# haesungpyun/seoul_tourism_recommendation_NGCF

Measured on AMD Instinct MI355X. Metric: NGCF 3-layer forward: propagated edges/sec + achieved HBM GB/s, d=128, higher is better.
Workload: dtype f32

## Files before the change

### seoul_tourism_recommendation_ngcf_amd/csrc/dense.hip

```cpp
#include "common.h"
#include <type_traits>

#ifndef NGCF_DC
#define NGCF_DC 16
#endif
#define NGCF_KC (2 * NGCF_DC)

typedef float f32x16 __attribute__((ext_vector_type(16)));
typedef float f32x4 __attribute__((ext_vector_type(4)));

__device__ __forceinline__ void pack_bias2(const float *__restrict__ b1, const float *__restrict__ b2, int d_out, int DOP,
                                           float *__restrict__ bias2)
{
    for (int j = threadIdx.x; j < DOP; j += 256) bias2[j] = j < d_out ? (b1[j] + b1[j]) + b2[j] : 0.f;
}

template <class T> __device__ __forceinline__ T tile_row(T base, int r, int lh) { return base + (r & 3) + 8 * (r >> 2) + 4 * lh; }

struct DenseAct {
    float leaky, drop_p, keep_scale;
    uint32_t drop_thr;
    uint64_t drop_seed;
    const float *drop_mask;
    int64_t ldm, n_rows;
// ... 156 lines not shown
        const int kl = idx / 32, w = idx % 32;
        Wt[((int64_t)chunk * NGCF_KC + kl) * DOP + g * 32 + w] = tile[kl][w];
    }
    if (blockIdx.x == 0) pack_bias2(b1, b2, d_out, DOP, bias2);
}

#ifndef NGCF_DENSE_WAVES_PER_EU
#define NGCF_DENSE_WAVES_PER_EU 1
#endif
template <int RW, int CW, int NT, bool ALIGNED, bool FAST>
__global__ __launch_bounds__(256, NGCF_DENSE_WAVES_PER_EU) void layer_dense_kernel(const float *__restrict__ LE, int64_t ldLE,
                                                          const float *__restrict__ Es, int64_t ldE, int64_t n_rows,
                                                          int d_in, int d_out, const float *__restrict__ Wt,
                                                          const float *__restrict__ bias2, int n_chunks,
                                                          float leaky, float drop_p, uint64_t drop_seed_in,
                                                          const float *__restrict__ drop_mask, int64_t ldm,
                                                          float *__restrict__ carry, int64_t ldc,
                                                          float *__restrict__ norm, int64_t ldn)
{
    const uint64_t drop_seed = drop_p > 0.f ? resolve_seed(drop_seed_in) : drop_seed_in;
    constexpr int BM = 32 * RW;
    constexpr int WCOLS = 32 * NT * CW;
    constexpr int XLD = NGCF_KC + 4;
    constexpr bool DB = WCOLS <= 128;
    constexpr int NBUF = DB ? 2 : 1;
    constexpr int SQ = NGCF_DC / 4;
    constexpr int RPP = 256 / SQ;
    constexpr int RR = (BM + RPP - 1) / RPP;
    constexpr int WF4 = NGCF_KC * WCOLS / 4;
    constexpr int WN = (WF4 + 255) / 256;
    __shared__ float Xs[NBUF * BM * XLD];
    __shared__ float Ws[NBUF * NGCF_KC * WCOLS];
    __shared__ float ssq[BM * CW];

    const int tid = threadIdx.x;
    const int wave = tid >> 6, lane = tid & 63;
    const int rw = wave / CW, cw = wave % CW;
    const int li = lane & 31, lh = lane >> 5;
    const int64_t row0 = (int64_t)blockIdx.x * BM;

    f32x16 acc[NT];
#pragma unroll
    for (int t = 0; t < NT; ++t)
#pragma unroll
        for (int r = 0; r < 16; ++r) acc[t][r] = 0.f;

    const int sq = tid % SQ;
    const int sr = tid / SQ;
    f32x4 xle[RR], xe[RR], wreg[WN];

    auto load_chunk = [&](int chunk) {
        const int c0 = chunk * NGCF_DC + sq * 4;
        if constexpr (FAST) {
            const int d4 = (d_in + 3) & ~3;
            const int cc = c0 < d4 ? c0 : d4 - 4;
            const bool k0 = c0 < d_in, k1 = c0 + 1 < d_in, k2 = c0 + 2 < d_in, k3 = c0 + 3 < d_in;
#pragma unroll
            for (int rr = 0; rr < RR; ++rr) {
                int64_t grow = row0 + (sr + rr * RPP) % BM;
                grow = grow < n_rows ? grow : n_rows - 1;
                f32x4 a = *reinterpret_cast<const f32x4 *>(LE + grow * ldLE + cc);
                f32x4 b = *reinterpret_cast<const f32x4 *>(Es + grow * ldE + cc);
                a.x = k0 ? a.x : 0.f; a.y = k1 ? a.y : 0.f; a.z = k2 ? a.z : 0.f; a.w = k3 ? a.w : 0.f;
                b.x = k0 ? b.x : 0.f; b.y = k1 ? b.y : 0.f; b.z = k2 ? b.z : 0.f; b.w = k3 ? b.w : 0.f;
                xle[rr] = a;
                xe[rr] = b;
            }
            const f32x4 *srcw = reinterpret_cast<const f32x4 *>(Wt + (int64_t)chunk * NGCF_KC * WCOLS);
#pragma unroll
            for (int i = 0; i < WN; ++i)
                if (WF4 % 256 == 0 || tid + i * 256 < WF4) wreg[i] = srcw[tid + i * 256];
            return;
        }
#pragma unroll
        for (int rr = 0; rr < RR; ++rr) {
            const int r = sr + rr * RPP;
            float le[4] = {0.f, 0.f, 0.f, 0.f}, e[4] = {0.f, 0.f, 0.f, 0.f};
            const int64_t grow = row0 + r;
            if (r < BM && grow < n_rows) {
                if (ALIGNED && c0 + 4 <= d_in) {
                    const float4 a = *reinterpret_cast<const float4 *>(LE + grow * ldLE + c0);
                    const float4 b = *reinterpret_cast<const float4 *>(Es + grow * ldE + c0);
                    le[0] = a.x; le[1] = a.y; le[2] = a.z; le[3] = a.w;
                    e[0] = b.x; e[1] = b.y; e[2] = b.z; e[3] = b.w;
                } else {
#pragma unroll
                    for (int q = 0; q < 4; ++q)
                        if (c0 + q < d_in) {
                            le[q] = LE[grow * ldLE + c0 + q];
                            e[q] = Es[grow * ldE + c0 + q];
                        }
                }
            }
            xle[rr] = f32x4{le[0], le[1], le[2], le[3]};
            xe[rr] = f32x4{e[0], e[1], e[2], e[3]};
        }
        const f32x4 *src = reinterpret_cast<const f32x4 *>(Wt + (int64_t)chunk * NGCF_KC * WCOLS);
#pragma unroll
        for (int i = 0; i < WN; ++i)
            if (WF4 % 256 == 0 || tid + i * 256 < WF4) wreg[i] = src[tid + i * 256];
    };
    auto store_chunk = [&](int buf) {
        float *X = Xs + buf * (BM * XLD);
#pragma unroll
        for (int rr = 0; rr < RR; ++rr) {
            const int r = sr + rr * RPP;
            if (r < BM) {
                const f32x4 a = xle[rr], b = xe[rr];
                *reinterpret_cast<f32x4 *>(X + r * XLD + sq * 4) = a + b;
                *reinterpret_cast<f32x4 *>(X + r * XLD + NGCF_DC + sq * 4) = a * b;
            }
        }
        f32x4 *dst = reinterpret_cast<f32x4 *>(Ws + buf * (NGCF_KC * WCOLS));
#pragma unroll
        for (int i = 0; i < WN; ++i)
            if (WF4 % 256 == 0 || tid + i * 256 < WF4) dst[tid + i * 256] = wreg[i];
    };
    auto compute_chunk = [&](int buf) {
        const float *X = Xs + buf * (BM * XLD) + (rw * 32 + li) * XLD + lh * 4;
        const float *W = Ws + buf * (NGCF_KC * WCOLS) + cw * (32 * NT) + li * NT;
#pragma unroll
        for (int kb = 0; kb < NGCF_KC / 8; ++kb) {
            const f32x4 a4 = *reinterpret_cast<const f32x4 *>(X + kb * 8);
#define NGCF_KSTEP(sx, aval)                                                                                   \
    {                                                                                                          \
        const float *wk = W + (kb * 8 + lh * 4 + sx) * WCOLS;                                                  \
        float bv[NT];                                                                                          \
        _Pragma("unroll") for (int t = 0; t < NT; ++t) bv[t] = wk[t];                                          \
        _Pragma("unroll") for (int t = 0; t < NT; ++t)                                                         \
            acc[t] = __builtin_amdgcn_mfma_f32_32x32x2f32(aval, bv[t], acc[t], 0, 0, 0);                       \
    }
            NGCF_KSTEP(0, a4.x) NGCF_KSTEP(1, a4.y) NGCF_KSTEP(2, a4.z) NGCF_KSTEP(3, a4.w)
#undef NGCF_KSTEP
        }
    };

    if (DB) {
        load_chunk(0);
        store_chunk(0);
        __syncthreads();
        for (int chunk = 0; chunk < n_chunks; ++chunk) {
            const bool more = chunk + 1 < n_chunks;
            if (more) load_chunk(chunk + 1);
            compute_chunk(chunk & 1);
            if (more) store_chunk((chunk + 1) & 1);
            __syncthreads();
        }
    } else {
        load_chunk(0);
        store_chunk(0);
        __syncthreads();
        for (int chunk = 0; chunk < n_chunks; ++chunk) {
            const bool more = chunk + 1 < n_chunks;
            if (more) load_chunk(chunk + 1);
            compute_chunk(0);
            __syncthreads();
            if (more) {
                store_chunk(0);
                __syncthreads();
            }
        }
    }

    const float keep_scale = drop_p > 0.f ? 1.f / (1.f - drop_p) : 1.f;
    const uint32_t drop_thr = msg_drop_thr(drop_p);
    float rowss[16];
#pragma unroll
    for (int r = 0; r < 16; ++r) rowss[r] = 0.f;
    if (!drop_mask && !(drop_p > 0.f)) {
#pragma unroll
        for (int t = 0; t < NT; ++t) {
            const int col = (cw * NT + t) * 32 + li;
            const float bz = bias2[col];
#pragma unroll
            for (int r = 0; r < 16; ++r) {
                float v = acc[t][r] + bz;
                v = v >= 0.f ? v : leaky * v;
                acc[t][r] = v;
                rowss[r] = fmaf(v, v, rowss[r]);
            }
        }
    } else {
#pragma unroll
        for (int t = 0; t < NT; ++t) {
            const int col = (cw * NT + t) * 32 + li;
            const float bz = bias2[col];
#pragma unroll
            for (int r = 0; r < 16; ++r) {
                float v = acc[t][r] + bz;
                v = v >= 0.f ? v : leaky * v;
                if (drop_mask) {
                    const int64_t grow = tile_row(row0 + rw * 32, r, lh);
                    v *= (grow < n_rows && col < d_out) ? drop_mask[grow * ldm + col] : 0.f;
                } else if (drop_p > 0.f) {
                    const int64_t grow = tile_row(row0 + rw * 32, r, lh);
                    v = msg_drop(v, drop_seed, grow, col, drop_thr, keep_scale);
                }
                acc[t][r] = v;
                rowss[r] = fmaf(v, v, rowss[r]);
            }
        }
    }
#pragma unroll
    for (int r = 0; r < 16; ++r) {
        float s = rowss[r];
        s += __shfl_xor(s, 1);
        s += __shfl_xor(s, 2);
        s += __shfl_xor(s, 4);
        s += __shfl_xor(s, 8);
        s += __shfl_xor(s, 16);
        rowss[r] = s;
    }
    if (CW > 1) {
        if (li == 0) {
#pragma unroll
            for (int r = 0; r < 16; ++r) {
                const int lr = tile_row(rw * 32, r, lh);
                ssq[lr * CW + cw] = rowss[r];
            }
        }
        __syncthreads();
#pragma unroll
        for (int r = 0; r < 16; ++r) {
            const int lr = tile_row(rw * 32, r, lh);
            float s = 0.f;
#pragma unroll
            for (int q = 0; q < CW; ++q) s += ssq[lr * CW + q];
            rowss[r] = s;
        }
    }
    if (row0 + BM <= n_rows && d_out == WCOLS) {
#pragma unroll
        for (int r = 0; r < 16; ++r) {
            const int64_t grow = tile_row(row0 + rw * 32, r, lh);
            const float inv = 1.f / fmaxf(sqrtf(rowss[r]), 1e-12f);
            float *nrow = norm + grow * ldn + cw * NT * 32 + li;
#pragma unroll
            for (int t = 0; t < NT; ++t) nrow[t * 32] = acc[t][r] * inv;
        }
        if (carry) {
#pragma unroll
            for (int r = 0; r < 16; ++r) {
                const int64_t grow = tile_row(row0 + rw * 32, r, lh);
                float *crow = carry + grow * ldc + cw * NT * 32 + li;
#pragma unroll
                for (int t = 0; t < NT; ++t) crow[t * 32] = acc[t][r];
            }
        }
        return;
    }
#pragma unroll
    for (int r = 0; r < 16; ++r) {
        const int64_t grow = tile_row(row0 + rw * 32, r, lh);
        if (grow >= n_rows) continue;
        const float nrm = fmaxf(sqrtf(rowss[r]), 1e-12f);
        const float inv = 1.f / nrm;
#pragma unroll
        for (int t = 0; t < NT; ++t) {
            const int col = (cw * NT + t) * 32 + li;
            if (col < d_out) {
                const float v = acc[t][r];
                if (carry) carry[grow * ldc + col] = v;
                norm[grow * ldn + col] = v * inv;
            }
        }
    }
}

constexpr int kResWaves = 8, kResWGs = 256;

typedef __bf16 bf16x8 __attribute__((ext_vector_type(8)));
typedef float f32x8 __attribute__((ext_vector_type(8)));

__device__ __forceinline__ void split3(f32x8 x, bf16x8 &h, bf16x8 &m, bf16x8 &l)
{
    h = __builtin_convertvector(x, bf16x8);
    const f32x8 r = x - __builtin_convertvector(h, f32x8);
    m = __builtin_convertvector(r, bf16x8);
    l = __builtin_convertvector(r - __builtin_convertvector(m, f32x8), bf16x8);
}

__global__ __launch_bounds__(256) void pack_weights_split_kernel(const float *__restrict__ W1, const float *__restrict__ b1,
                                                                 const float *__restrict__ W2, const float *__restrict__ b2,
                                                                 int d_in, int d_out, int n_chunks, bf16x8 *__restrict__ Whm,
                                                                 bf16x8 *__restrict__ Wl, float *__restrict__ bias2)
{
    const int idx = blockIdx.x * 256 + threadIdx.x;
    if (idx < n_chunks * 512) {
        const int lane = idx & 63, frag = idx >> 6, t = frag & 3, s = (frag >> 2) & 1, c = frag >> 3;
        const int col = t * 32 + (lane & 31), in0 = c * NGCF_DC + 8 * (lane >> 5);
        const float *w = (s ? W2 : W1) + (int64_t)col * d_in;
        f32x8 x;
#pragma unroll
        for (int j = 0; j < 8; ++j) x[j] = (col < d_out && in0 + j < d_in) ? w[in0 + j] : 0.f;
        bf16x8 h, m, l;
        split3(x, h, m, l);
        Whm[(frag * 2 + 0) * 64 + lane] = h;
        Whm[(frag * 2 + 1) * 64 + lane] = m;
        Wl[idx] = l;
    }
    if (blockIdx.x == 0) pack_bias2(b1, b2, d_out, 128, bias2);
}

template <bool SPLIT>
__device__ __forceinline__ void dense_persistent_tiles(const float *LE, int64_t ldLE, const float *Es, int64_t ldE, int64_t n_rows,
                                                       int d_in, int d_out, const f32x4 *w_lds, const bf16x8 *Wl, const float *bias2,
                                                       int n_chunks, float leaky, float drop_p, uint64_t drop_seed_in,
                                                       const float *drop_mask, int64_t ldm, float *carry, int64_t ldc, float *norm,
                                                       int64_t ldn)
{
    const uint64_t drop_seed = drop_p > 0.f ? resolve_seed(drop_seed_in) : drop_seed_in;
    constexpr int NT = 4, WCOLS = 128;
    constexpr int CA = SPLIT ? 8 : 4, CB = SPLIT ? 4 : 8;
    using AFrag = std::conditional_t<SPLIT, bf16x8[2][3], f32x4[4]>;
    constexpr int NL = SPLIT ? 8 : 1;
    extern __shared__ f32x4 Wres[];
    const int tid = threadIdx.x, wave = tid >> 6, lane = tid & 63;
    const int li = lane & 31, lh = lane >> 5;
    for (int i = tid; i < n_chunks * 1024; i += kResWaves * 64) Wres[i] = w_lds[i];
    __syncthreads();
    const int64_t n_tiles = (n_rows + 31) / 32;
    const int d4 = (d_in + 3) & ~3;
    float bz[NT];
#pragma unroll
    for (int t = 0; t < NT; ++t) bz[t] = bias2[t * 32 + li];
    const int last = n_chunks - 1;
    const int64_t tile_step = (int64_t)gridDim.x * kResWaves;
    auto row_of = [&](int64_t t) {
        int64_t g = t * 32 + li;
        return g < n_rows ? g : n_rows - 1;
    };
    auto fetch = [&](const float *le_row, const float *e_row, int c, f32x4 &la, f32x4 &lb, f32x4 &ea, f32x4 &eb) {
        const int ca = c * NGCF_DC + lh * CA;
        fetch_pieces(le_row, e_row, ca, ca + CB, d4, la, lb, ea, eb);
    };
    auto fetch_l = [&](int c, bf16x8 (&bl)[NL]) {
        if constexpr (SPLIT) {
#pragma unroll
            for (int f = 0; f < 8; ++f) bl[f] = Wl[(c * 8 + f) * 64 + lane];
        }
    };
    f32x4 la0, lb0, ea0, eb0, la1, lb1, ea1, eb1;
    bf16x8 bl0[NL], bl1[NL];
    auto fetch_tile = [&](int64_t t) {
        const int64_t g = row_of(t);
        fetch(LE + g * ldLE, Es + g * ldE, 0, la0, lb0, ea0, eb0);
        fetch(LE + g * ldLE, Es + g * ldE, last < 1 ? last : 1, la1, lb1, ea1, eb1);
    };
    fetch_l(0, bl0);
    int64_t tile = (int64_t)blockIdx.x * kResWaves + wave;
    fetch_tile(tile < n_tiles ? tile : 0);
    for (; tile < n_tiles; tile += tile_step) {
        const int64_t row0 = tile * 32;
        const int64_t grow_l = row_of(tile);
        const float *le_row = LE + grow_l * ldLE, *e_row = Es + grow_l * ldE;
        f32x16 acc[NT];
#pragma unroll
        for (int t = 0; t < NT; ++t)
#pragma unroll
            for (int r = 0; r < 16; ++r) acc[t][r] = 0.f;
        auto form = [&](int c, f32x4 la, f32x4 lb, f32x4 ea, f32x4 eb, AFrag &a) {
            const int ca = c * NGCF_DC + lh * CA;
            zero_tail(ca, ca + CB, d_in, la, lb, ea, eb);
            const f32x4 sa = la + ea, sb = lb + eb, pa = la * ea, pb = lb * eb;
            if constexpr (SPLIT) {
                split3(__builtin_shufflevector(sa, sb, 0, 1, 2, 3, 4, 5, 6, 7), a[0][0], a[0][1], a[0][2]);
                split3(__builtin_shufflevector(pa, pb, 0, 1, 2, 3, 4, 5, 6, 7), a[1][0], a[1][1], a[1][2]);
            } else {
                a[0] = sa, a[1] = sb, a[2] = pa, a[3] = pb;
            }
        };
        auto chunk_mfma = [&](int c, const AFrag &a, const bf16x8 (&bl)[NL]) {
            if constexpr (SPLIT) {
                const bf16x8 *wc = reinterpret_cast<const bf16x8 *>(Wres) + c * 1024 + lane;
#pragma unroll
                for (int s = 0; s < 2; ++s) {
                    const bf16x8 &ah = a[s][0], &am = a[s][1], &al = a[s][2];
#pragma unroll
                    for (int t = 0; t < NT; ++t) {
                        const bf16x8 bh = wc[((s * 4 + t) * 2 + 0) * 64], bm = wc[((s * 4 + t) * 2 + 1) * 64];
                        acc[t] = __builtin_amdgcn_mfma_f32_32x32x16_bf16(am, bm, acc[t], 0, 0, 0);
                        acc[t] = __builtin_amdgcn_mfma_f32_32x32x16_bf16(al, bh, acc[t], 0, 0, 0);
                        acc[t] = __builtin_amdgcn_mfma_f32_32x32x16_bf16(ah, bl[s * 4 + t], acc[t], 0, 0, 0);
                        acc[t] = __builtin_amdgcn_mfma_f32_32x32x16_bf16(am, bh, acc[t], 0, 0, 0);
                        acc[t] = __builtin_amdgcn_mfma_f32_32x32x16_bf16(ah, bm, acc[t], 0, 0, 0);
                        acc[t] = __builtin_amdgcn_mfma_f32_32x32x16_bf16(ah, bh, acc[t], 0, 0, 0);
                    }
                }
            } else {
                const float *wc = reinterpret_cast<const float *>(Wres) + li * NT + (int64_t)c * NGCF_KC * WCOLS;
#pragma unroll
                for (int kb = 0; kb < 4; ++kb) {
#pragma unroll
                    for (int sx = 0; sx < 4; ++sx) {
                        const f32x4 bv = *reinterpret_cast<const f32x4 *>(wc + (kb * 8 + lh * 4 + sx) * WCOLS);
                        acc[0] = __builtin_amdgcn_mfma_f32_32x32x2f32(a[kb][sx], bv.x, acc[0], 0, 0, 0);
                        acc[1] = __builtin_amdgcn_mfma_f32_32x32x2f32(a[kb][sx], bv.y, acc[1], 0, 0, 0);
                        acc[2] = __builtin_amdgcn_mfma_f32_32x32x2f32(a[kb][sx], bv.z, acc[2], 0, 0, 0);
                        acc[3] = __builtin_amdgcn_mfma_f32_32x32x2f32(a[kb][sx], bv.w, acc[3], 0, 0, 0);
                    }
                }
            }
        };
        int c = 0;
        for (; c + 1 < n_chunks; c += 2) {
            {
                AFrag a;
                form(c, la0, lb0, ea0, eb0, a);
                fetch(le_row, e_row, c + 2 < last ? c + 2 : last, la0, lb0, ea0, eb0);
                fetch_l(c + 1, bl1);
                __builtin_amdgcn_sched_barrier(0);
                chunk_mfma(c, a, bl0);
            }
            {
                AFrag a;
                form(c + 1, la1, lb1, ea1, eb1, a);
                fetch(le_row, e_row, c + 3 < last ? c + 3 : last, la1, lb1, ea1, eb1);
                fetch_l(c + 2 < last ? c + 2 : last, bl0);
                __builtin_amdgcn_sched_barrier(0);
                chunk_mfma(c + 1, a, bl1);
            }
        }
        if (c < n_chunks) {
            AFrag a;
            form(c, la0, lb0, ea0, eb0, a);
            chunk_mfma(c, a, bl0);
        }
        fetch_tile(tile + tile_step < n_tiles ? tile + tile_step : tile);
        fetch_l(0, bl0);
        __builtin_amdgcn_sched_barrier(0);
        if constexpr (!SPLIT) {
            const DenseAct act(leaky, drop_p, drop_seed, drop_mask, ldm, n_rows, d_out);
            const WaveTile w{row0, 0, 0, li, lh};
            const bool full = row0 + 32 <= n_rows && d_out == WCOLS;
            dense_epilogue<1, NT, true>(acc, [&](int t, int) { return bz[t]; }, act, w, nullptr, full, carry, ldc, norm, ldn);
        } else {
            const float keep_scale = drop_p > 0.f ? 1.f / (1.f - drop_p) : 1.f;
            const uint32_t drop_thr = msg_drop_thr(drop_p);
            float rowss[16];
#pragma unroll
            for (int r = 0; r < 16; ++r) rowss[r] = 0.f;
            const bool any_drop = drop_mask || drop_p > 0.f;
            if (!any_drop) {
#pragma unroll
                for (int t = 0; t < NT; ++t)
#pragma unroll
                    for (int r = 0; r < 16; ++r) {
                        float v = acc[t][r] + bz[t];
                        v = v >= 0.f ? v : leaky * v;
                        acc[t][r] = v;
                        rowss[r] = fmaf(v, v, rowss[r]);
                    }
            } else {
#pragma unroll
                for (int t = 0; t < NT; ++t) {
                    const int col = t * 32 + li;
#pragma unroll
                    for (int r = 0; r < 16; ++r) {
                        float v = acc[t][r] + bz[t];
                        v = v >= 0.f ? v : leaky * v;
                        const int64_t grow = tile_row(row0, r, lh);
                        if (drop_mask) v *= (grow < n_rows && col < d_out) ? drop_mask[grow * ldm + col] : 0.f;
                        else v = msg_drop(v, drop_seed, grow, col, drop_thr, keep_scale);
                        acc[t][r] = v;
                        rowss[r] = fmaf(v, v, rowss[r]);
                    }
                }
            }
#pragma unroll
            for (int r = 0; r < 16; ++r) {
                float s2 = rowss[r];
                s2 += __shfl_xor(s2, 1);
                s2 += __shfl_xor(s2, 2);
                s2 += __shfl_xor(s2, 4);
                s2 += __shfl_xor(s2, 8);
                s2 += __shfl_xor(s2, 16);
                rowss[r] = s2;
            }
            if (row0 + 32 <= n_rows && d_out == WCOLS) {
#pragma unroll
                for (int r = 0; r < 16; ++r) {
                    const int64_t grow = tile_row(row0, r, lh);
                    const float inv = 1.f / fmaxf(sqrtf(rowss[r]), 1e-12f);
                    float *nrow = norm + grow * ldn + li;
#pragma unroll
                    for (int t = 0; t < NT; ++t) nrow[t * 32] = acc[t][r] * inv;
                }
                if (carry) {
#pragma unroll
                    for (int r = 0; r < 16; ++r) {
                        float *crow = carry + tile_row(row0, r, lh) * ldc + li;
#pragma unroll
                        for (int t = 0; t < NT; ++t) crow[t * 32] = acc[t][r];
                    }
                }
                continue;
            }
#pragma unroll
            for (int r = 0; r < 16; ++r) {
                const int64_t grow = tile_row(row0, r, lh);
                if (grow >= n_rows) continue;
                const float inv = 1.f / fmaxf(sqrtf(rowss[r]), 1e-12f);
#pragma unroll
                for (int t = 0; t < NT; ++t) {
                    const int col = t * 32 + li;
                    if (col < d_out) {
                        const float v = acc[t][r];
                        if (carry) carry[grow * ldc + col] = v;
                        norm[grow * ldn + col] = v * inv;
                    }
                }
            }
        }
    }
}

__global__ __launch_bounds__(kResWaves * 64) void layer_dense_resident_kernel(
    const float *__restrict__ LE, int64_t ldLE, const float *__restrict__ Es, int64_t ldE, int64_t n_rows, int d_in, int d_out,
    const float *__restrict__ Wt, const float *__restrict__ bias2, int n_chunks, float leaky, float drop_p, uint64_t drop_seed_in,
    const float *__restrict__ drop_mask, int64_t ldm, float *__restrict__ carry, int64_t ldc, float *__restrict__ norm, int64_t ldn)
{
    dense_persistent_tiles<false>(LE, ldLE, Es, ldE, n_rows, d_in, d_out, reinterpret_cast<const f32x4 *>(Wt), nullptr, bias2,
                                  n_chunks, leaky, drop_p, drop_seed_in, drop_mask, ldm, carry, ldc, norm, ldn);
}

__global__ __launch_bounds__(kResWaves * 64) void layer_dense_split_kernel(
    const float *__restrict__ LE, int64_t ldLE, const float *__restrict__ Es, int64_t ldE, int64_t n_rows, int d_in, int d_out,
    const bf16x8 *__restrict__ Whm, const bf16x8 *__restrict__ Wl, const float *__restrict__ bias2, int n_chunks, float leaky,
    float drop_p, uint64_t drop_seed_in, const float *__restrict__ drop_mask, int64_t ldm, float *__restrict__ carry, int64_t ldc,
    float *__restrict__ norm, int64_t ldn)
{
    dense_persistent_tiles<true>(LE, ldLE, Es, ldE, n_rows, d_in, d_out, reinterpret_cast<const f32x4 *>(Whm), Wl, bias2, n_chunks,
                                 leaky, drop_p, drop_seed_in, drop_mask, ldm, carry, ldc, norm, ldn);
}


typedef float f32x2 __attribute__((ext_vector_type(2)));
template <int NT> struct TileVec;
template <> struct TileVec<4> { using type = f32x4; };
template <> struct TileVec<2> { using type = f32x2; };

template <int CW, int NT>
__global__ __launch_bounds__(CW * 64) void layer_dense_direct_kernel(
    const float *__restrict__ LE, int64_t ldLE, const float *__restrict__ Es, int64_t ldE, int64_t n_rows, int d_in, int d_out,
    const float *__restrict__ Wt, const float *__restrict__ bias2, int n_chunks, float leaky, float drop_p, uint64_t drop_seed_in,
    const float *__restrict__ drop_mask, int64_t ldm, float *__restrict__ carry, int64_t ldc, float *__restrict__ norm, int64_t ldn)
{
    const uint64_t drop_seed = drop_p > 0.f ? resolve_seed(drop_seed_in) : drop_seed_in;
    constexpr int WCOLS = 32 * NT * CW;
    using BV = typename TileVec<NT>::type;
    __shared__ float ssq[32 * CW];
    const int tid = threadIdx.x, cw = tid >> 6, lane = tid & 63;
    const int li = lane & 31, lh = lane >> 5;
    const int64_t row0 = (int64_t)blockIdx.x * 32;
    int64_t grow_l = row0 + li;
    grow_l = grow_l < n_rows ? grow_l : n_rows - 1;
    const float *le_row = LE + grow_l * ldLE, *e_row = Es + grow_l * ldE;
    const int d4 = (d_in + 3) & ~3;
    const float *Wl = Wt + (int64_t)lh * 4 * WCOLS + cw * (32 * NT) + li * NT;
    f32x16 acc[NT];
#pragma unroll
    for (int t = 0; t < NT; ++t)
#pragma unroll
        for (int r = 0; r < 16; ++r) acc[t][r] = 0.f;
    auto fetch_a = [&](int c, f32x4 &la, f32x4 &lb, f32x4 &ea, f32x4 &eb) {
        const int ca = c * NGCF_DC + lh * 4;
        fetch_pieces(le_row, e_row, ca, ca + 8, d4, la, lb, ea, eb);
    };
    auto fetch_b = [&](int c, BV (&b)[16]) {
        const float *wc = Wl + (int64_t)c * NGCF_KC * WCOLS;
#pragma unroll
        for (int q = 0; q < 16; ++q) b[q] = *reinterpret_cast<const BV *>(wc + ((q >> 2) * 8 + (q & 3)) * WCOLS);
    };
    auto form = [&](int c, f32x4 la, f32x4 lb, f32x4 ea, f32x4 eb, f32x4 (&a4)[4]) {
        const int ca = c * NGCF_DC + lh * 4;
        zero_tail(ca, ca + 8, d_in, la, lb, ea, eb);
        a4[0] = la + ea, a4[1] = lb + eb, a4[2] = la * ea, a4[3] = lb * eb;
    };
    auto chunk_mfma = [&](const f32x4 (&a4)[4], const BV (&b)[16]) {
#pragma unroll
        for (int kb = 0; kb < 4; ++kb)
#pragma unroll
            for (int sx = 0; sx < 4; ++sx) {
                const BV bv = b[kb * 4 + sx];
#pragma unroll
                for (int t = 0; t < NT; ++t) acc[t] = __builtin_amdgcn_mfma_f32_32x32x2f32(a4[kb][sx], bv[t], acc[t], 0, 0, 0);
            }
    };
    const int last = n_chunks - 1;
    f32x4 la0, lb0, ea0, eb0, la1, lb1, ea1, eb1;
    BV b0[16], b1[16];
    fetch_a(0, la0, lb0, ea0, eb0);
    fetch_b(0, b0);
    fetch_a(last < 1 ? last : 1, la1, lb1, ea1, eb1);
    fetch_b(last < 1 ? last : 1, b1);
    int c = 0;
    for (; c + 1 < n_chunks; c += 2) {
        {
            f32x4 a4[4];
            form(c, la0, lb0, ea0, eb0, a4);
            fetch_a(c + 2 < last ? c + 2 : last, la0, lb0, ea0, eb0);
            __builtin_amdgcn_sched_barrier(0);
            chunk_mfma(a4, b0);
            fetch_b(c + 2 < last ? c + 2 : last, b0);
            __builtin_amdgcn_sched_barrier(0);
        }
        {
            f32x4 a4[4];
            form(c + 1, la1, lb1, ea1, eb1, a4);
            fetch_a(c + 3 < last ? c + 3 : last, la1, lb1, ea1, eb1);
            __builtin_amdgcn_sched_barrier(0);
            chunk_mfma(a4, b1);
            fetch_b(c + 3 < last ? c + 3 : last, b1);
            __builtin_amdgcn_sched_barrier(0);
        }
    }
    if (c < n_chunks) {
        f32x4 a4[4];
        form(c, la0, lb0, ea0, eb0, a4);
        chunk_mfma(a4, b0);
    }
    const DenseAct act(leaky, drop_p, drop_seed, drop_mask, ldm, n_rows, d_out);
    float bz[NT];
#pragma unroll
    for (int t = 0; t < NT; ++t) bz[t] = bias2[(cw * NT + t) * 32 + li];
    const WaveTile w{row0, cw * NT * 32, cw, li, lh};
    dense_epilogue<CW, NT, false>(acc, [&](int t, int) { return bz[t]; }, act, w, ssq, false, carry, ldc, norm, ldn);
}

constexpr int kTallRows = 96;

__global__ __launch_bounds__(256) void pack_weights_tall_kernel(const float *__restrict__ W1, const float *__restrict__ b1,
                                                                const float *__restrict__ W2, const float *__restrict__ b2, int d_in,
                                                                int d_out, int DOP, float *__restrict__ Wp, float *__restrict__ bias2)
{
    __shared__ float tile[NGCF_KC][33];
    const int n_ct = DOP / 32;
    const int chunk = blockIdx.x / n_ct, ct = blockIdx.x % n_ct;
    for (int idx = threadIdx.x; idx < 32 * NGCF_KC; idx += 256) {
        const int j = idx / NGCF_KC, kl = idx % NGCF_KC;
        const int oc = ct * 32 + j, col = chunk * NGCF_DC + (kl % NGCF_DC);
        float v = 0.f;
        if (oc < d_out && col < d_in) v = (kl < NGCF_DC ? W1 : W2)[(int64_t)oc * d_in + col];
        tile[kl][j] = v;
    }
    __syncthreads();
    float *dst = Wp + ((int64_t)chunk * n_ct + ct) * (32 * NGCF_KC);
    for (int idx = threadIdx.x; idx < 32 * NGCF_KC; idx += 256) {
        const int sx = idx & 3, li = (idx >> 2) & 31, lh = (idx >> 7) & 1, kb = idx >> 8;
        dst[idx] = tile[kb * 8 + lh * 4 + sx][li];
    }
    if (blockIdx.x == 0) pack_bias2(b1, b2, d_out, DOP, bias2);
}

__global__ __launch_bounds__(256) void layer_dense_tall_kernel(
    const float *__restrict__ LE, int64_t ldLE, const float *__restrict__ Es, int64_t ldE, int64_t n_rows, int d_in, int d_out,
    const float *__restrict__ Wp, const float *__restrict__ bias2, int n_chunks, int n_ct, float leaky, float drop_p,
    uint64_t drop_seed_in, const float *__restrict__ drop_mask, int64_t ldm, float *__restrict__ carry, int64_t ldc,
    float *__restrict__ norm, int64_t ldn)
{
    const uint64_t drop_seed = drop_p > 0.f ? resolve_seed(drop_seed_in) : drop_seed_in;
    constexpr int XLD = NGCF_KC + 4;
    constexpr int MT = kTallRows / 32;
    constexpr int XBUF = kTallRows * XLD;
    __shared__ float Xs[3 * XBUF];
    const int tid = threadIdx.x, wave = tid >> 6, lane = tid & 63;
    const int li = lane & 31, lh = lane >> 5;
    const int n_cp = n_ct / 4;
    const int64_t row0 = (int64_t)(blockIdx.x / n_cp) * kTallRows;
    const int ct = (blockIdx.x % n_cp) * 4 + wave;
    const int d4 = (d_in + 3) & ~3;
    const bool two = tid < 384 - 256;
    int64_t grow_a = row0 + (tid >> 2), grow_b = row0 + 64 + (tid >> 2);
    grow_a = grow_a < n_rows ? grow_a : n_rows - 1;
    grow_b = two ? (grow_b < n_rows ? grow_b : n_rows - 1) : grow_a;
    const int sq4 = (tid & 3) * 4;
    const float *le_a = LE + grow_a * ldLE + sq4, *e_a = Es + grow_a * ldE + sq4, *le_b = LE + grow_b * ldLE + sq4, *e_b = Es + grow_b * ldE + sq4;
    const int last = n_chunks - 1;
    const int cc_last = (last * NGCF_DC + sq4 < d4 ? last * NGCF_DC + sq4 : d4 - 4) - sq4;
    struct XRegs { f32x4 al, ae, bl, be; };
    XRegs x0, x1;
    auto load_x = [&](int c, XRegs &x) {
        const int off = c < last ? c * NGCF_DC : cc_last;
        x.al = *reinterpret_cast<const f32x4 *>(le_a + off);
        x.ae = *reinterpret_cast<const f32x4 *>(e_a + off);
        x.bl = *reinterpret_cast<const f32x4 *>(le_b + off);
        x.be = *reinterpret_cast<const f32x4 *>(e_b + off);
    };
    float *xs_w = Xs + (tid >> 2) * XLD + sq4;
    auto store_x = [&](int c, int buf, XRegs x) {
        if (c == last) {
            const int c0 = c * NGCF_DC + sq4;
#pragma unroll
            for (int q = 0; q < 4; ++q)
                if (c0 + q >= d_in) x.al[q] = 0.f, x.ae[q] = 0.f, x.bl[q] = 0.f, x.be[q] = 0.f;
        }
        float *xr = xs_w + buf * XBUF;
        *reinterpret_cast<f32x4 *>(xr) = x.al + x.ae;
        *reinterpret_cast<f32x4 *>(xr + NGCF_DC) = x.al * x.ae;
        if (two) {
            *reinterpret_cast<f32x4 *>(xr + 64 * XLD) = x.bl + x.be;
            *reinterpret_cast<f32x4 *>(xr + 64 * XLD + NGCF_DC) = x.bl * x.be;
        }
    };
    const float *wl = Wp + (int64_t)ct * (32 * NGCF_KC) + lane * 4;
    const int64_t wstep = (int64_t)n_ct * (32 * NGCF_KC);
    f32x4 b0[4], b1[4];
    auto load_b = [&](int c, f32x4 (&b)[4]) {
        const float *w = wl + (int64_t)c * wstep;
#pragma unroll
        for (int kb = 0; kb < 4; ++kb) b[kb] = *reinterpret_cast<const f32x4 *>(w + kb * 256);
    };
    f32x16 acc[MT];
#pragma unroll
    for (int m = 0; m < MT; ++m)
#pragma unroll
        for (int r = 0; r < 16; ++r) acc[m][r] = 0.f;
    const float *xs_r = Xs + li * XLD + lh * 4;
    auto read_a = [&](int buf, int kb, f32x4 (&a)[MT]) {
#pragma unroll
        for (int m = 0; m < MT; ++m)
            a[m] = *reinterpret_cast<const f32x4 *>(xs_r + buf * XBUF + m * 32 * XLD + (kb >> 1) * NGCF_DC + (kb & 1) * 8);
    };
    auto cl = [&](int c) { return c < last ? c : last; };
    f32x4 an[MT];
    auto step = [&](int c, int buf, const f32x4 (&b)[4], XRegs &x) {
        f32x4 a0[MT], a1[MT];
#pragma unroll
        for (int m = 0; m < MT; ++m) a0[m] = an[m];
#pragma unroll
        for (int kb = 0; kb < 4; kb += 2) {
            read_a(buf, kb + 1, a1);
            __builtin_amdgcn_sched_barrier(0);
#pragma unroll
            for (int sx = 0; sx < 4; ++sx)
#pragma unroll
                for (int m = 0; m < MT; ++m) acc[m] = __builtin_amdgcn_mfma_f32_32x32x2f32(a0[m][sx], b[kb][sx], acc[m], 0, 0, 0);
            if (kb + 2 < 4) read_a(buf, kb + 2, a0);
            else {
                const int b2 = buf >= 1 ? buf - 1 : 2;
                store_x(cl(c + 2), b2, x);
                load_x(cl(c + 4), x);
                read_a(buf == 2 ? 0 : buf + 1, 0, an);
            }
            __builtin_amdgcn_sched_barrier(0);
#pragma unroll
            for (int sx = 0; sx < 4; ++sx)
#pragma unroll
                for (int m = 0; m < MT; ++m) acc[m] = __builtin_amdgcn_mfma_f32_32x32x2f32(a1[m][sx], b[kb + 1][sx], acc[m], 0, 0, 0);
        }
    };
    load_x(0, x0);
    load_b(0, b0);
    load_x(cl(1), x1);
    load_b(cl(1), b1);
    store_x(0, 0, x0);
    load_x(cl(2), x0);
    store_x(cl(1), 1, x1);
    load_x(cl(3), x1);
    __syncthreads();
    read_a(0, 0, an);
    int buf = 0;
    int c = 0;
    for (; c + 1 < n_chunks; c += 2) {
        step(c, buf, b0, x0);
        load_b(cl(c + 2), b0);
        __syncthreads();
        buf = buf == 2 ? 0 : buf + 1;
        step(c + 1, buf, b1, x1);
        load_b(cl(c + 3), b1);
        __syncthreads();
        buf = buf == 2 ? 0 : buf + 1;
    }
    if (c < n_chunks) step(c, buf, b0, x0);
    const float keep_scale = drop_p > 0.f ? 1.f / (1.f - drop_p) : 1.f;
    const uint32_t drop_thr = msg_drop_thr(drop_p);
    const int col = ct * 32 + li;
    const float bz = bias2[col];
    if (col >= d_out) return;
#pragma unroll
    for (int m = 0; m < MT; ++m)
#pragma unroll
        for (int r = 0; r < 16; ++r) {
            const int64_t grow = tile_row(row0 + m * 32, r, lh);
            if (grow >= n_rows) continue;
            float v = acc[m][r] + bz;
            v = v >= 0.f ? v : leaky * v;
            if (drop_mask) v *= drop_mask[grow * ldm + col];
            else if (drop_p > 0.f) {
                v = msg_drop(v, drop_seed, grow, col, drop_thr, keep_scale);
            }
            if (carry) carry[grow * ldc + col] = v;
            norm[grow * ldn + col] = v;
        }
}

template <int CW>
__global__ __launch_bounds__(256) void row_scale_kernel(float *__restrict__ norm, int64_t ldn, int64_t n_rows, int d_out)
{
    const int lane = threadIdx.x & 63, li = lane & 31, half = lane >> 5;
    const int64_t row = (int64_t)blockIdx.x * 4 + (threadIdx.x >> 6);
    if (row >= n_rows) return;
    float *x = norm + row * ldn;
    constexpr int PP = CW / 2;
    float v[PP][4], part[PP];
#pragma unroll
    for (int p = 0; p < PP; ++p) {
        const int cw = half + 2 * p;
        float s = 0.f;
#pragma unroll
        for (int t = 0; t < 4; ++t) {
            const int col = cw * 128 + t * 32 + li;
            v[p][t] = col < d_out ? x[col] : 0.f;
            s = fmaf(v[p][t], v[p][t], s);
        }
        s += __shfl_xor(s, 1);
        s += __shfl_xor(s, 2);
        s += __shfl_xor(s, 4);
        s += __shfl_xor(s, 8);
        s += __shfl_xor(s, 16);
        part[p] = s;
    }
    float other[PP];
#pragma unroll
    for (int p = 0; p < PP; ++p) other[p] = __shfl_xor(part[p], 32);
    float ss = 0.f;
#pragma unroll
    for (int p = 0; p < PP; ++p) {
        const float even = half == 0 ? part[p] : other[p], odd = half == 0 ? other[p] : part[p];
        ss += even;
        ss += odd;
    }
    const float inv = 1.f / fmaxf(sqrtf(ss), 1e-12f);
#pragma unroll
    for (int p = 0; p < PP; ++p)
#pragma unroll
        for (int t = 0; t < 4; ++t) {
            const int col = (half + 2 * p) * 128 + t * 32 + li;
            if (col < d_out) x[col] = v[p][t] * inv;
        }
}

static int dense_dop(int d_out)
{
    if (d_out <= 32) return 32;
    if (d_out <= 64) return 64;
    if (d_out <= 96) return 96;
    if (d_out <= 128) return 128;
    if (d_out <= 256) return 256;
    if (d_out <= 512) return 512;
    return -1;
}

extern "C" int64_t ngcf_dense_workspace_bytes(int d_in, int d_out)
{
    int dop = dense_dop(d_out);
    if (dop < 0 || d_in <= 0) return -1;
    dop = std::max(dop, 128);
    const int64_t n_chunks = (d_in + NGCF_DC - 1) / NGCF_DC;
    const int64_t fp32_packed = (n_chunks * NGCF_KC * dop + dop) * (int64_t)sizeof(float);
    const int64_t split_packed = 128 * (int64_t)sizeof(float) + n_chunks * 3 * 8 * 1024;
    return align_up(std::max(fp32_packed, split_packed), 256) + 256;
}

struct DenseCall {
    const float *LE;
    int64_t ldLE;
    const float *Es;
    int64_t ldE, n_rows;
    int d_in, d_out;
    float leaky, drop_p;
    uint64_t drop_seed;
    const float *drop_mask;
    int64_t ldm;
    float *carry;
    int64_t ldc;
    float *norm;
    int64_t ldn;
    hipStream_t stream;
    template <class Kernel, class... W> void launch(Kernel kernel, int64_t grid, int block, size_t lds, W... w) const
    {
        kernel<<<dim3((unsigned)grid), block, lds, stream>>>(LE, ldLE, Es, ldE, n_rows, d_in, d_out, w..., leaky, drop_p, drop_seed, drop_mask,
                                                             ldm, carry, ldc, norm, ldn);
    }
};

template <int RW, int CW, int NT>
static void launch_staged(const DenseCall &k, bool al, bool padded, const float *Wt, const float *bias2, int n_chunks)
{
    const int64_t blocks = (k.n_rows + 32 * RW - 1) / (32 * RW);
    if (padded) k.launch(layer_dense_kernel<RW, CW, NT, true, true>, blocks, 256, 0, Wt, bias2, n_chunks);
    else if (al) k.launch(layer_dense_kernel<RW, CW, NT, true, false>, blocks, 256, 0, Wt, bias2, n_chunks);
    else k.launch(layer_dense_kernel<RW, CW, NT, false, false>, blocks, 256, 0, Wt, bias2, n_chunks);
}

enum DenseKernel { kDenseTall, kDenseSplit, kDenseResident, kDenseDirect, kDenseStaged };
struct DensePath {
    DenseKernel kernel;
    int dop;
    bool small_rows;
    bool al;
    bool padded;
    int tile;
    const char *name;
};
static DensePath dense_path(int64_t n_rows, int d_in, int d_out, const float *LE, int64_t ldLE, const float *Es, int64_t ldEs)
{
    DensePath p{};
    p.dop = dense_dop(d_out);
    p.small_rows = p.dop <= 128 && n_rows <= 16384 && ngcf_opts().dense_small_tiles;
    if (p.small_rows) p.dop = 128;
    const int dop = p.dop;
    p.al = (ldLE % 4 == 0) && (ldEs % 4 == 0) && aligned16(LE) && aligned16(Es);
    p.padded = p.al && ldLE >= align_up(d_in, 4) && ldEs >= align_up(d_in, 4) && d_in >= 4;
    const int n_chunks = (d_in + NGCF_DC - 1) / NGCF_DC;

    const int tall_env = ngcf_opts().dense_tall;
    const bool tall_pays = dop == 512 ? (n_rows <= 6144 || n_rows > 8192) : (n_rows > 8192 && n_rows <= 131072);
    if (tall_env && dop >= 256 && p.padded && (tall_pays || tall_env == 2)) {
        p.kernel = kDenseTall;
        p.name = dop == 256 ? "tall256" : "tall512";
        return p;
    }

    const int resident = ngcf_opts().dense_resident;
    const int64_t lds_bytes = (int64_t)n_chunks * NGCF_KC * 128 * (int64_t)sizeof(float);
    const bool resident_fits = resident && dop == 128 && p.padded && lds_bytes <= 150 * 1024 &&
                               n_rows >= (int64_t)ngcf_opts().dense_resident_min_rows;
    if (resident_fits) {
        p.kernel = resident == 4 ? kDenseSplit : kDenseResident;
        p.name = resident == 4 ? "split" : "resident";
        return p;
    }

    const int direct_env = ngcf_opts().dense_direct;
    if (direct_env && dop >= 256 && p.padded && (n_rows <= 8192 || direct_env == 2)) {
        p.kernel = kDenseDirect;
        p.name = dop == 256 ? "direct<2,4>" : "direct<4,4>";
        return p;
    }

#define NGCF_STAGED_NAMES(cfg) {"staged" cfg "/unaligned", "staged" cfg "/aligned", "staged" cfg "/padded"}
    static const char *const names[7][3] = {NGCF_STAGED_NAMES("<1,4,1>"), NGCF_STAGED_NAMES("<4,1,1>"), NGCF_STAGED_NAMES("<4,1,2>"),
                                            NGCF_STAGED_NAMES("<4,1,3>"), NGCF_STAGED_NAMES("<4,1,4>"), NGCF_STAGED_NAMES("<2,2,4>"),
                                            NGCF_STAGED_NAMES("<1,4,4>")};
#undef NGCF_STAGED_NAMES
    p.kernel = kDenseStaged;
    p.tile = p.small_rows ? 0 : dop <= 128 ? dop / 32 : dop == 256 ? 5 : 6;
    p.name = names[p.tile][p.padded ? 2 : p.al ? 1 : 0];
    return p;
}

extern "C" const char *ngcf_dense_path(int64_t n_rows, int d_in, int d_out, const float *LE, int64_t ldLE, const float *Es, int64_t ldEs)
{
    if (n_rows < 0 || d_in <= 0 || d_out <= 0 || dense_dop(d_out) < 0 || ldLE < d_in || ldEs < d_in) {
        fail(NGCF_ERR_ARG, "dense_path: bad sizes");
        return nullptr;
    }
    return dense_path(n_rows, d_in, d_out, LE, ldLE, Es, ldEs).name;
}

extern "C" int ngcf_layer_dense_f32(const float *LE, int64_t ldLE, const float *Es, int64_t ldEs, int64_t n_rows,
                                    int d_in, const float *W1, const float *b1, const float *W2, const float *b2,
                                    int d_out, float leaky, float drop_p, uint64_t drop_seed, const float *drop_mask,
                                    int64_t ld_mask, float *carry, int64_t ldc, float *norm, int64_t ldn, void *workspace,
                                    int64_t workspace_bytes, void *stream_)
{
    hipStream_t stream = (hipStream_t)stream_;
    if (!LE || !Es || !W1 || !b1 || !W2 || !b2 || !norm) return fail(NGCF_ERR_ARG, "layer_dense: null argument");
    if (n_rows < 0 || d_in <= 0 || d_out <= 0) return fail(NGCF_ERR_ARG, "layer_dense: bad sizes");
    if (dense_dop(d_out) < 0) return fail(NGCF_ERR_ARG, "layer_dense: d_out=%d > 512 is not supported", d_out);
    if (!(drop_p >= 0.f && drop_p < 1.f)) return fail(NGCF_ERR_ARG, "layer_dense: drop_p=%f not in [0,1)", drop_p);
    if (ldLE < d_in || ldEs < d_in || ldn < d_out || (carry && ldc < d_out) || (drop_mask && ld_mask < d_out))
        return fail(NGCF_ERR_ARG, "layer_dense: leading dimension too small");
    const int64_t need = ngcf_dense_workspace_bytes(d_in, d_out);
    if (!workspace || workspace_bytes < need)
        return fail(NGCF_ERR_WORKSPACE, "layer_dense: workspace %lld B < %lld B", (long long)workspace_bytes, (long long)need);
    if (n_rows == 0) return NGCF_OK;
    const DensePath path = dense_path(n_rows, d_in, d_out, LE, ldLE, Es, ldEs);
    const int dop = path.dop;
    const int n_chunks = (d_in + NGCF_DC - 1) / NGCF_DC;
    float *Wt = reinterpret_cast<float *>(align_up((int64_t)(uintptr_t)workspace, 256));
    float *bias2 = Wt + (int64_t)n_chunks * NGCF_KC * dop;
    const DenseCall call{LE, ldLE, Es, ldEs, n_rows, d_in, d_out, leaky, drop_p, drop_seed, drop_mask, ld_mask, carry, ldc, norm, ldn, stream};

    if (path.kernel == kDenseTall) {
        const int n_ct = dop / 32;
        pack_weights_tall_kernel<<<dim3((unsigned)(n_chunks * n_ct)), 256, 0, stream>>>(W1, b1, W2, b2, d_in, d_out, dop, Wt, bias2);
        LAUNCH_CHECK();
        const int64_t groups = (n_rows + kTallRows - 1) / kTallRows;
        call.launch(layer_dense_tall_kernel, groups * (n_ct / 4), 256, 0, Wt, bias2, n_chunks, n_ct);
        LAUNCH_CHECK();
        if (dop == 256) row_scale_kernel<2><<<dim3((unsigned)((n_rows + 3) / 4)), 256, 0, stream>>>(norm, ldn, n_rows, d_out);
        else row_scale_kernel<4><<<dim3((unsigned)((n_rows + 3) / 4)), 256, 0, stream>>>(norm, ldn, n_rows, d_out);
        LAUNCH_CHECK();
        return NGCF_OK;
    }

    const int64_t lds_bytes = (int64_t)n_chunks * NGCF_KC * 128 * (int64_t)sizeof(float);
    auto pack_fp32 = [&](int nt) {
        pack_weights_kernel<<<dim3((unsigned)(n_chunks * (dop / 32))), 256, 0, stream>>>(W1, b1, W2, b2, d_in, d_out, n_chunks, dop,
                                                                                        nt, Wt, bias2);
        return hipGetLastError();
    };
    if (path.kernel == kDenseSplit) {
        HIP_TRY(allow_full_lds<layer_dense_split_kernel>());
        float *sbias = Wt;
        bf16x8 *whm = reinterpret_cast<bf16x8 *>(Wt + 128);
        bf16x8 *wl = whm + (int64_t)n_chunks * 1024;
        pack_weights_split_kernel<<<dim3((unsigned)(n_chunks * 2)), 256, 0, stream>>>(W1, b1, W2, b2, d_in, d_out, n_chunks,
                                                                                      whm, wl, sbias);
        LAUNCH_CHECK();
        call.launch(layer_dense_split_kernel, kResWGs, kResWaves * 64, (size_t)n_chunks * 16 * 1024, whm, wl, sbias, n_chunks);
        LAUNCH_CHECK();
        return NGCF_OK;
    }
    if (path.kernel == kDenseResident) {
        HIP_TRY(pack_fp32(4));
        HIP_TRY(allow_full_lds<layer_dense_resident_kernel>());
        call.launch(layer_dense_resident_kernel, kResWGs, kResWaves * 64, (size_t)lds_bytes, Wt, bias2, n_chunks);
        LAUNCH_CHECK();
        return NGCF_OK;
    }

    HIP_TRY(pack_fp32(path.small_rows ? 1 : dop <= 128 ? dop / 32 : 4));
    if (path.kernel == kDenseDirect) {
        const int64_t blocks = (n_rows + 31) / 32;
        if (dop == 256) call.launch(layer_dense_direct_kernel<2, 4>, blocks, 128, 0, Wt, bias2, n_chunks);
        else call.launch(layer_dense_direct_kernel<4, 4>, blocks, 256, 0, Wt, bias2, n_chunks);
        LAUNCH_CHECK();
        return NGCF_OK;
    }

#define NGCF_DENSE(RW, CW, NT) launch_staged<RW, CW, NT>(call, path.al, path.padded, Wt, bias2, n_chunks)
    switch (path.tile) {
    case 0: NGCF_DENSE(1, 4, 1); break;
    case 1: NGCF_DENSE(4, 1, 1); break;
    case 2: NGCF_DENSE(4, 1, 2); break;
    case 3: NGCF_DENSE(4, 1, 3); break;
    case 4: NGCF_DENSE(4, 1, 4); break;
    case 5: NGCF_DENSE(2, 2, 4); break;
    default: NGCF_DENSE(1, 4, 4);
    }
#undef NGCF_DENSE
    LAUNCH_CHECK();
    return NGCF_OK;
}

extern "C" int64_t ngcf_layer_workspace_bytes(const ngcf_csr_t *c, int d_in, int d_out)
{
    if (!c) return -1;
    const int64_t a = ngcf_spmm_workspace_bytes(c, d_in);
    const int64_t b = ngcf_dense_workspace_bytes(d_in, d_out);
    if (a < 0 || b < 0) return -1;
    const int64_t le = align_up(c->n_rows * align_up(d_in, 32) * (int64_t)sizeof(float), 256);
    return a + b + le + 256;
}

extern "C" int ngcf_layer_fused_f32(const ngcf_csr_t *c, const float *Eg, int64_t ldEg, const float *Es, int64_t ldEs,
                                    int d_in, const float *W1, const float *b1, const float *W2, const float *b2,
                                    int d_out, float leaky, float drop_p, uint64_t drop_seed, const float *drop_mask,
                                    int64_t ld_mask, float *carry, int64_t ldc, float *norm, int64_t ldn, void *workspace,
                                    int64_t workspace_bytes, void *stream)
{
    if (!c) return fail(NGCF_ERR_ARG, "layer_fused: null csr");
    const int64_t need = ngcf_layer_workspace_bytes(c, d_in, d_out);
    if (need < 0) return fail(NGCF_ERR_ARG, "layer_fused: unsupported widths d_in=%d d_out=%d", d_in, d_out);
    if (!workspace || workspace_bytes < need)
        return fail(NGCF_ERR_WORKSPACE, "layer_fused: workspace %lld B < %lld B", (long long)workspace_bytes, (long long)need);
    char *ws = reinterpret_cast<char *>(align_up((int64_t)(uintptr_t)workspace, 256));
    const int64_t ldLE = align_up(d_in, 32);
    float *LE = reinterpret_cast<float *>(ws);
    ws += align_up(c->n_rows * ldLE * (int64_t)sizeof(float), 256);
    const int64_t spmm_ws = ngcf_spmm_workspace_bytes(c, d_in);
    void *ws_spmm = ws;
    ws += spmm_ws;
    const int64_t dense_ws = ngcf_dense_workspace_bytes(d_in, d_out);
    void *ws_dense = ws;
    const int d_sp = ngcf_spmm_product_width(c, Eg, ldEg, d_in);
    int rc = ngcf_spmm_csr_f32(c, Eg, ldEg, d_sp, LE, ldLE, ws_spmm, spmm_ws, stream);
    if (rc != NGCF_OK) return rc;
    return ngcf_layer_dense_f32(LE, ldLE, Es, ldEs, c->n_rows, d_in, W1, b1, W2, b2, d_out, leaky, drop_p, drop_seed,
                                drop_mask, ld_mask, carry, ldc, norm, ldn, ws_dense, dense_ws, stream);
}
```

Before: 28.46 billion.

## Dedicate a store wave in split dense kernel fed by LDS ring buffer

In the split (bf16x3) dense kernel, one wave per workgroup is turned into a dedicated store wave. Compute waves stage normalized-output tiles (8 rows x 128 floats plus inverse norms) into an LDS ring of slots, using an atomic ticket counter and per-slot sequence flags. The store wave drains those slots into norm and carry with 128-bit vectorized stores. This aims to overlap global stores with MFMA compute and to coalesce writes, at the cost of one fewer compute wave, extra LDS usage, and spin-wait synchronization overhead.

```diff
diff --git a/seoul_tourism_recommendation_ngcf_amd/csrc/dense.hip b/seoul_tourism_recommendation_ngcf_amd/csrc/dense.hip
--- a/seoul_tourism_recommendation_ngcf_amd/csrc/dense.hip
+++ b/seoul_tourism_recommendation_ngcf_amd/csrc/dense.hip
@@ -482,6 +482,86 @@
     if (blockIdx.x == 0) pack_bias2(b1, b2, d_out, 128, bias2);
 }
 
+constexpr int kSplitStoreWaves = 1, kSplitComputeWaves = kResWaves - kSplitStoreWaves;
+constexpr int kSlotFloats = 8 * 128, kSlotMeta = 12;
+constexpr uint32_t kStageSpinLimit = 1u << 22;
+__host__ __device__ inline int split_stage_slots(int n_chunks) { return n_chunks <= 8 ? 7 : 3; }
+__host__ __device__ inline size_t split_lds_bytes(int n_chunks)
+{
+    const int ns = split_stage_slots(n_chunks);
+    return (size_t)n_chunks * 16 * 1024 + (size_t)ns * kSlotFloats * sizeof(float) + (4 + (size_t)ns * kSlotMeta) * sizeof(uint32_t);
+}
+struct SplitStage {
+    float *data;
+    uint32_t *meta;
+    int ns;
+    __device__ __forceinline__ SplitStage(void *after_weights, int n_chunks)
+        : data(static_cast<float *>(after_weights)), ns(split_stage_slots(n_chunks))
+    {
+        meta = reinterpret_cast<uint32_t *>(data + ns * kSlotFloats);
+    }
+    __device__ __forceinline__ uint32_t slot_of(uint32_t ticket) const { return ns == 7 ? ticket % 7u : ticket % 3u; }
+    __device__ __forceinline__ uint32_t *slot_meta(uint32_t slot) const { return meta + 4 + slot * kSlotMeta; }
+    __device__ __forceinline__ void init(int tid) const
+    {
+        if (tid == 0) meta[0] = 0;
+        if (tid < ns) slot_meta(tid)[0] = tid;
+    }
+    __device__ __forceinline__ void wait_for(const uint32_t *seq, uint32_t want) const
+    {
+        for (uint32_t n = 0; __hip_atomic_load(seq, __ATOMIC_RELAXED, __HIP_MEMORY_SCOPE_WORKGROUP) != want && n < kStageSpinLimit; ++n)
+            __builtin_amdgcn_s_sleep(1);
+        __builtin_amdgcn_fence(__ATOMIC_ACQUIRE, "workgroup");
+    }
+    __device__ __forceinline__ void publish(uint32_t *seq, uint32_t value, int lane) const
+    {
+        __builtin_amdgcn_fence(__ATOMIC_RELEASE, "workgroup");
+        if (lane == 0) __hip_atomic_store(seq, value, __ATOMIC_RELAXED, __HIP_MEMORY_SCOPE_WORKGROUP);
+    }
+};
+
+__device__ __forceinline__ void split_store_wave(const SplitStage &st, uint32_t first, uint32_t total, int lane, int64_t n_rows,
+                                                 int d_out, float *carry, int64_t ldc, float *norm, int64_t ldn)
+{
+    const int li = lane & 31, lh = lane >> 5, col = li * 4;
+    const bool vec = (reinterpret_cast<uintptr_t>(norm) & 15) == 0 && (ldn & 3) == 0 &&
+                     (!carry || ((reinterpret_cast<uintptr_t>(carry) & 15) == 0 && (ldc & 3) == 0));
+    for (uint32_t ticket = first; ticket < total; ticket += kSplitStoreWaves) {
+        const uint32_t slot = st.slot_of(ticket);
+        uint32_t *m = st.slot_meta(slot);
+        st.wait_for(m, ticket + 1);
+        const int64_t row0 = *reinterpret_cast<const int64_t *>(m + 2);
+        const float *d = st.data + slot * kSlotFloats;
+        f32x4 v[4];
+        float inv[4];
+#pragma unroll
+        for (int q = 0; q < 4; ++q) {
+            const int j = 2 * q + lh;
+            v[q] = *reinterpret_cast<const f32x4 *>(d + j * 128 + (col ^ ((j >> 2) * 32)));
+            inv[q] = reinterpret_cast<const float *>(m + 4)[j];
+        }
+        st.publish(m, ticket + st.ns, lane);
+#pragma unroll
+        for (int q = 0; q < 4; ++q) {
+            const int64_t row = row0 + 2 * q + lh;
+            if (row >= n_rows) continue;
+            const f32x4 nv = v[q] * inv[q];
+            float *nrow = norm + row * ldn + col;
+            if (vec && col + 4 <= d_out) {
+                *reinterpret_cast<f32x4 *>(nrow) = nv;
+                if (carry) *reinterpret_cast<f32x4 *>(carry + row * ldc + col) = v[q];
+            } else {
+#pragma unroll
+                for (int e = 0; e < 4; ++e)
+                    if (col + e < d_out) {
+                        nrow[e] = nv[e];
+                        if (carry) carry[row * ldc + col + e] = v[q][e];
+                    }
+            }
+        }
+    }
+}
+
 template <bool SPLIT>
 __device__ __forceinline__ void dense_persistent_tiles(const float *LE, int64_t ldLE, const float *Es, int64_t ldE, int64_t n_rows,
                                                        int d_in, int d_out, const f32x4 *w_lds, const bf16x8 *Wl, const float *bias2,
@@ -497,15 +577,31 @@
     extern __shared__ f32x4 Wres[];
     const int tid = threadIdx.x, wave = tid >> 6, lane = tid & 63;
     const int li = lane & 31, lh = lane >> 5;
+    constexpr int NC = SPLIT ? kSplitComputeWaves : kResWaves;
     for (int i = tid; i < n_chunks * 1024; i += kResWaves * 64) Wres[i] = w_lds[i];
+    const SplitStage stage(Wres + n_chunks * 1024, n_chunks);
+    if constexpr (SPLIT) stage.init(tid);
     __syncthreads();
     const int64_t n_tiles = (n_rows + 31) / 32;
+    const int64_t tile_step = (int64_t)gridDim.x * NC;
+    auto first_tile = [&](int w) { return SPLIT ? blockIdx.x + (int64_t)gridDim.x * w : (int64_t)blockIdx.x * NC + w; };
+    if constexpr (SPLIT) {
+        if (wave >= NC) {
+            int64_t tiles = 0;
+            for (int w = 0; w < NC; ++w) {
+                const int64_t t0 = first_tile(w);
+                if (t0 < n_tiles) tiles += (n_tiles - 1 - t0) / tile_step + 1;
+            }
+            __builtin_amdgcn_s_setprio(3);
+            split_store_wave(stage, wave - NC, (uint32_t)(4 * tiles), lane, n_rows, d_out, carry, ldc, norm, ldn);
+            return;
+        }
+    }
     const int d4 = (d_in + 3) & ~3;
     float bz[NT];
 #pragma unroll
     for (int t = 0; t < NT; ++t) bz[t] = bias2[t * 32 + li];
     const int last = n_chunks - 1;
-    const int64_t tile_step = (int64_t)gridDim.x * kResWaves;
     auto row_of = [&](int64_t t) {
         int64_t g = t * 32 + li;
         return g < n_rows ? g : n_rows - 1;
@@ -528,7 +624,7 @@
         fetch(LE + g * ldLE, Es + g * ldE, last < 1 ? last : 1, la1, lb1, ea1, eb1);
     };
     fetch_l(0, bl0);
-    int64_t tile = (int64_t)blockIdx.x * kResWaves + wave;
+    int64_t tile = first_tile(wave);
     fetch_tile(tile < n_tiles ? tile : 0);
     for (; tile < n_tiles; tile += tile_step) {
         const int64_t row0 = tile * 32;
@@ -657,39 +753,26 @@
                 s2 += __shfl_xor(s2, 16);
                 rowss[r] = s2;
             }
-            if (row0 + 32 <= n_rows && d_out == WCOLS) {
-#pragma unroll
-                for (int r = 0; r < 16; ++r) {
-                    const int64_t grow = tile_row(row0, r, lh);
-                    const float inv = 1.f / fmaxf(sqrtf(rowss[r]), 1e-12f);
-                    float *nrow = norm + grow * ldn + li;
-#pragma unroll
-                    for (int t = 0; t < NT; ++t) nrow[t * 32] = acc[t][r] * inv;
+#pragma unroll
+            for (int g = 0; g < 4; ++g) {
+                uint32_t ticket = 0;
+                if (lane == 0) ticket = __hip_atomic_fetch_add(stage.meta, 1u, __ATOMIC_RELAXED, __HIP_MEMORY_SCOPE_WORKGROUP);
+                ticket = __builtin_amdgcn_readfirstlane(ticket);
+                const uint32_t slot = stage.slot_of(ticket);
+                uint32_t *m = stage.slot_meta(slot);
+                stage.wait_for(m, ticket);
+                float *d = stage.data + slot * kSlotFloats + 4 * lh * 128 + li;
+                float inv_l = 0.f;
+#pragma unroll
+                for (int rr = 0; rr < 4; ++rr) {
+                    const float inv = 1.f / fmaxf(sqrtf(rowss[4 * g + rr]), 1e-12f);
+                    inv_l = li == rr ? inv : inv_l;
+#pragma unroll
+                    for (int t = 0; t < NT; ++t) d[rr * 128 + (t ^ lh) * 32] = acc[t][4 * g + rr];
                 }
-                if (carry) {
-#pragma unroll
-                    for (int r = 0; r < 16; ++r) {
-                        float *crow = carry + tile_row(row0, r, lh) * ldc + li;
-#pragma unroll
-                        for (int t = 0; t < NT; ++t) crow[t * 32] = acc[t][r];
-                    }
-                }
-                continue;
-            }
-#pragma unroll
-            for (int r = 0; r < 16; ++r) {
-                const int64_t grow = tile_row(row0, r, lh);
-                if (grow >= n_rows) continue;
-                const float inv = 1.f / fmaxf(sqrtf(rowss[r]), 1e-12f);
-#pragma unroll
-                for (int t = 0; t < NT; ++t) {
-                    const int col = t * 32 + li;
-                    if (col < d_out) {
-                        const float v = acc[t][r];
-                        if (carry) carry[grow * ldc + col] = v;
-                        norm[grow * ldn + col] = v * inv;
-                    }
-                }
+                if (li < 4) reinterpret_cast<float *>(m + 4)[li + 4 * lh] = inv_l;
+                if (lane == 0) *reinterpret_cast<int64_t *>(m + 2) = row0 + 8 * g;
+                stage.publish(m, ticket + 1, lane);
             }
         }
     }
@@ -1191,7 +1274,7 @@
         pack_weights_split_kernel<<<dim3((unsigned)(n_chunks * 2)), 256, 0, stream>>>(W1, b1, W2, b2, d_in, d_out, n_chunks,
                                                                                       whm, wl, sbias);
         LAUNCH_CHECK();
-        call.launch(layer_dense_split_kernel, kResWGs, kResWaves * 64, (size_t)n_chunks * 16 * 1024, whm, wl, sbias, n_chunks);
+        call.launch(layer_dense_split_kernel, kResWGs, kResWaves * 64, split_lds_bytes(n_chunks), whm, wl, sbias, n_chunks);
         LAUNCH_CHECK();
         return NGCF_OK;
     }
```

Measured after the change: 27.93 billion. 1.9% lower.
